# JiQi-da/Mixed-Graph-ADMM

Hardware: AMD Instinct MI355X
Metric: ADMM iters/sec x batch (sample-iterations/s) (higher is better)
Workload: dtype f32; 1 GPU; cfg2: PEMS04-shaped synthetic graph N=307 (path+chords, 340 edges), kNN k=4, T=24, t_in=12; batch_per_gpu=4096, global_batch=4096, ablation=None, graph=kNN-directed, max_cg_iter=100, parallelism=batch-sharded x1, no collective on the convergence path, final RCCL gather, all_finite=True

## Files before the change

include/mgadmm.h:

```cpp
#ifndef MGADMM_H
#define MGADMM_H

#include <stdint.h>

#ifdef __cplusplus
extern "C" {
#endif

typedef enum {
    MGADMM_OK = 0,
    MGADMM_ERR_INVALID = -1,
    MGADMM_ERR_HIP = -2,
    MGADMM_ERR_NONFINITE = -3,
    MGADMM_ERR_UNSUPPORTED = -4,
    MGADMM_ERR_NOMEM = -5
} mgadmm_status;

typedef enum { MGADMM_F32 = 0, MGADMM_F64 = 1 } mgadmm_dtype_t;

typedef enum {
    MGADMM_TEMPORAL_SPATIAL = 0,
    MGADMM_TEMPORAL_BAND = 1
} mgadmm_temporal_mode_t;

// ... 28 lines not shown
    const float* u_val;
    const int32_t* d_rowptr;
    const int32_t* d_col;
    const float* d_val;
    int32_t transpose_by_gather;
    int32_t q1_identity_t0;
    int32_t skip;
    const float* band_w;
    int32_t reorder;
    int32_t device;
} mgadmm_graph_desc;

typedef struct {
    double rho, rho_u, rho_d, mu_u, mu_d1, mu_d2;
    int32_t t_in;
    int32_t ablation;
    double cg_tol;
    int32_t max_cg_iter;
    double admm_tol;
    int32_t max_admm_iter;
    int32_t dtype;
    int32_t check_stop;
    int32_t path;
    int32_t record_cg_coeffs;
    int32_t cg_convergence;
    int32_t max_inner_iter;
    int32_t admm_convergence;
} mgadmm_params;

typedef struct {
    int32_t n_iters;
    double* metrics;
    double* delta_x_per_step;
    int32_t* cg_iters;
    double* metrics_per_sample;
    double* cg_alpha;
    double* cg_beta;
    int32_t* n_iters_per_sample;
} mgadmm_history;

typedef struct {
    void* zu; void* zd; void* phi; void* gamma; void* gamma_u; void* gamma_d;
} mgadmm_state;

typedef struct mgadmm_graph mgadmm_graph;
typedef struct mgadmm_solver mgadmm_solver;

const char* mgadmm_version(void);
const char* mgadmm_last_error(void);

int mgadmm_graph_create(const mgadmm_graph_desc* desc, mgadmm_graph** out);
int mgadmm_graph_destroy(mgadmm_graph* g);
int mgadmm_graph_transpose_nnz(const mgadmm_graph* g, int32_t* nnz);
int mgadmm_graph_get_transpose(const mgadmm_graph* g, int32_t* rowptr, int32_t* col, float* val);
int mgadmm_graph_get_perm(const mgadmm_graph* g, int32_t* perm);

int mgadmm_solver_create(mgadmm_graph* g, const mgadmm_params* p, int32_t max_batch, mgadmm_solver** out);
int mgadmm_solver_destroy(mgadmm_solver* s);
int mgadmm_solver_set_params(mgadmm_solver* s, const mgadmm_params* p);
typedef struct {
    const double *rho, *rho_u, *rho_d, *mu_u, *mu_d1, *mu_d2;
} mgadmm_sample_params;
int mgadmm_solver_set_sample_params(mgadmm_solver* s, const mgadmm_sample_params* sp, int32_t B);
int64_t mgadmm_solver_workspace_bytes(const mgadmm_solver* s);
int mgadmm_solver_path(const mgadmm_solver* s, int32_t B);

typedef enum {
    MGADMM_Q_LDS_OK = 0,
    MGADMM_Q_LDS_TPG = 1,
    MGADMM_Q_LDS_THREADS = 2,
    MGADMM_Q_LDS_BYTES = 3,
    MGADMM_Q_LDS_ROW_STRIDE = 4,
    MGADMM_Q_NNZ_U = 5,
    MGADMM_Q_NNZ_D = 6,
    MGADMM_Q_NNZ_DT = 7,
    MGADMM_Q_TILE_ROWS = 8,
    MGADMM_Q_LDS_UNIFORM = 9,
    MGADMM_Q_LDS_TAIL_PAIRS = 10,
    MGADMM_Q_LDS_LEAD = 11,
    MGADMM_Q_LDS_SLOTS = 12,
    MGADMM_Q_LDS_CHUNK = 13,
    MGADMM_Q_LDS_ROWS = 14,
    MGADMM_Q_CLDR_SLOTS = 15,
    MGADMM_Q_LDS_INSTANCE = 16
} mgadmm_query_t;
int mgadmm_solver_query(const mgadmm_solver* s, int32_t what, int64_t* out);

int mgadmm_apply(mgadmm_solver* s, int32_t op, const void* x, void* y, int32_t B, void* stream);
int mgadmm_lhs(mgadmm_solver* s, int32_t which, const void* x, const void* mask, void* y, int32_t B, void* stream);
int mgadmm_phi_direct(mgadmm_solver* s, const void* x, const void* gamma, void* phi, int32_t B, void* stream);
int mgadmm_initial_guess(mgadmm_solver* s, const void* y, void* x, int32_t B, void* stream);
int mgadmm_initial_interpolation(mgadmm_solver* s, const void* y, const void* mask, int32_t mask_is_f32,
                                 void* x, int32_t B, void* stream);
int mgadmm_cg(mgadmm_solver* s, int32_t which, const void* rhs, const void* x0, const void* mask, void* x,
              int32_t* iters, double* alpha, double* beta, int32_t B, void* stream);
int mgadmm_solve(mgadmm_solver* s, const void* y, const void* mask, int32_t mask_is_f32, int32_t B, void* x_out,
                 const mgadmm_state* state_out, mgadmm_history* hist, void* stream);

int mgadmm_solve_from(mgadmm_solver* s, const void* y, const void* mask, int32_t mask_is_f32, int32_t B, const void* x0,
                      const mgadmm_state* state_in, void* x_out, const mgadmm_state* state_out, mgadmm_history* hist,
                      void* stream);
int mgadmm_two_loops(mgadmm_solver* s, const void* y, const void* mask, int32_t mask_is_f32, int32_t B, void* x_out,
                     const mgadmm_state* state_out, mgadmm_history* hist, void* stream);

int mgadmm_knn_graph(int32_t n_nodes, int64_t n_edges, const int64_t* edges, const double* dists, int32_t k,
                     int32_t* nn_out, float* nd_out, int32_t device);
int mgadmm_weight_tables(int32_t n_nodes, int32_t k1, const int64_t* connect_list, const float* dist_list,
                         double u_sigma, double d_sigma, int32_t regularized, float* u_ew, float* d_ew,
                         double* sigmas_out, int32_t device);

int mgadmm_series_stats(const void* series, int64_t n_steps, int32_t n_cols, int32_t dtype, void* o_min, void* o_max,
                        void* o_mean, void* o_std, void* stream);
int mgadmm_series_affine(void* series, int64_t n_steps, int32_t n_cols, int32_t dtype, const void* shift, const void* scale,
                         const void* scale_lo, int32_t inverse, void* stream);
int mgadmm_gather_windows(const void* series, int64_t n_steps, int32_t n_cols, int32_t dtype, const int64_t* starts, int32_t B,
                          int32_t win, const float* mask, void* out, void* stream);

#define MGADMM_NPROF 4
int mgadmm_prof_begin(mgadmm_solver* s);
int mgadmm_prof_end(mgadmm_solver* s, int64_t* counts , double* total_ms ,
                    double* bytes );

#ifdef __cplusplus
}
#endif
#endif
```

mixed-graph-admm_amd/csrc/engine.h:

```cpp
#pragma once
#include <math.h>
#include <cmath>
#include <stdlib.h>
#include <string.h>

#include <algorithm>
#include <type_traits>

#include "common.h"
#include "cldr_tiles.h"
#include "stream_kernels.h"
#include "lds_args.h"
#include "lds_banks.h"
#include "lds_rows.h"

namespace {

struct LhsDef {
    int kind;
    int hth;
    double c1, c2;
};

enum VecId {
// ... 480 lines not shown
    }

    int set_sample_params(const mgadmm_sample_params* sp, int B) override {
        if (sp == nullptr || B == 0) {
            sp_B = 0;
            for (auto& v : sp_val) v.clear();
            return MGADMM_OK;
        }
        MG_REQUIRE(B >= 1 && B <= Bmax, "set_sample_params: batch %d outside [1, max_batch=%d]", B, Bmax);
        static const char* const names[6] = {"rho", "rho_u", "rho_d", "mu_u", "mu_d1", "mu_d2"};
        const double* const src[6] = {sp->rho, sp->rho_u, sp->rho_d, sp->mu_u, sp->mu_d1, sp->mu_d2};
        for (int f = 0; f < 6; ++f) {
            if (!src[f]) continue;
            for (int b = 0; b < B; ++b) {
                const double v = src[f][b];
                MG_REQUIRE(std::isfinite(v), "set_sample_params: %s[%d] is not finite", names[f], b);
                if (f < 3) MG_REQUIRE(v > 0.0, "set_sample_params: %s[%d] = %g, should be > 0", names[f], b, v);
                else MG_REQUIRE(v >= 0.0, "set_sample_params: %s[%d] = %g, should be >= 0", names[f], b, v);
            }
        }
        for (int f = 0; f < 6; ++f) {
            if (src[f]) sp_val[f].assign(src[f], src[f] + B);
            else sp_val[f].clear();
        }
        sp_B = B;
        MG_HIP(hipSetDevice(g->device));
        return upload_sample_params();
    }

    int upload_sample_params() {
        std::vector<LdsSampleParams> rec((size_t)sp_B);
        const double scalar[6] = {p.rho, p.rho_u, p.rho_d, p.mu_u, p.mu_d1, p.mu_d2};
        for (int b = 0; b < sp_B; ++b) {
            double w[6];
            for (int f = 0; f < 6; ++f) w[f] = sp_val[f].empty() ? scalar[f] : sp_val[f][(size_t)b];
            const LhsDef dx = lhs_def_of(MGADMM_LHS_X, p.ablation, w[0], w[1], w[2], w[3], w[5]);
            LdsSampleParams& r = rec[(size_t)b];
            r.cx1 = (float)dx.c1; r.cx2 = (float)dx.c2;
            r.rho = (float)w[0]; r.rho_u = (float)w[1]; r.rho_d = (float)w[2];
            r.mu_u = (float)w[3]; r.mu_d1 = (float)w[4]; r.mu_d2 = (float)w[5];
        }
        if (!d_sp) MG_HIP(hipMalloc(&d_sp, sizeof(LdsSampleParams) * (size_t)Bmax));
        MG_HIP(hipMemcpy(d_sp, rec.data(), sizeof(LdsSampleParams) * rec.size(), hipMemcpyHostToDevice));
        return MGADMM_OK;
    }

    int check_sample_params(int B) const {
        MG_REQUIRE(B == sp_B, "solve: the sample_params table holds %d samples, the solve has B = %d", sp_B, B);
        const char* why = nullptr;
        if (!std::is_same<S, float>::value) why = "float64 arithmetic runs on the streaming path";
        else if (p.path == MGADMM_PATH_STREAM) why = "path is MGADMM_PATH_STREAM";
        else if (p.cg_convergence == MGADMM_CG_BATCH_MAX) why = "cg_convergence batch_max runs on the streaming path";
        else if (!lds.ok) why = "the LDS-resident path cannot hold this graph (it needs T*N*8 B + tables <= 160 KiB and N*G <= 1024)";
        if (why) {
            mg_set_error("solve: sample_params (per-sample ADMM weights) are implemented by the LDS-resident float32 path only: %s", why);
            return MGADMM_ERR_UNSUPPORTED;
        }
        if (p.check_stop && p.admm_convergence == MGADMM_ADMM_WHOLE_BATCH) {
            mg_set_error("solve: sample_params with check_stop need admm_convergence per_sample (the whole_batch stop test would sum "
                         "the residuals of different problems); or run a fixed count with check_stop = 0");
            return MGADMM_ERR_UNSUPPORTED;
        }
        return MGADMM_OK;
    }

    int64_t workspace_bytes() const override { return ws_bytes; }
    int path_for(int) const override { return use_lds() ? MGADMM_PATH_LDS : MGADMM_PATH_STREAM; }
    bool use_lds() const { return lds.ok && p.path != MGADMM_PATH_STREAM && p.cg_convergence == MGADMM_CG_PER_SAMPLE; }
    int query(int what, int64_t* out) const override {
        switch (what) {
            case MGADMM_Q_LDS_OK: *out = lds.ok ? 1 : 0; break;
            case MGADMM_Q_LDS_TPG: *out = lds.TPG; break;
            case MGADMM_Q_LDS_THREADS: *out = lds.nthreads; break;
            case MGADMM_Q_LDS_BYTES: *out = (int64_t)lds.lds_bytes; break;
            case MGADMM_Q_LDS_ROW_STRIDE: *out = lds.TS; break;
            case MGADMM_Q_LDS_UNIFORM: *out = lds.uniform45; break;
            case MGADMM_Q_LDS_TAIL_PAIRS: *out = lds.tail_pairs; break;
            case MGADMM_Q_LDS_LEAD: *out = LDS_NLEAD; break;
            case MGADMM_Q_LDS_SLOTS: *out = lds.slots; break;
            case MGADMM_Q_LDS_CHUNK: *out = std::max(1, std::min(lds_chunk, LDS_MAXJ_POOL)); break;
            case MGADMM_Q_LDS_ROWS: *out = lds.NR; break;
            case MGADMM_Q_CLDR_SLOTS: *out = cldr_dev.state == 1 ? cl_gt : 0; break;
            case MGADMM_Q_LDS_INSTANCE: *out = lds_instance; break;
            case MGADMM_Q_NNZ_U: *out = g->hWu.nnz(); break;
            case MGADMM_Q_NNZ_D: *out = g->hWd.nnz(); break;
            case MGADMM_Q_NNZ_DT: *out = g->hWdT.nnz(); break;
            case MGADMM_Q_TILE_ROWS: {
                TileGeom tg;
                *out = make_tile_geom(make_geom(Bmax), tg) ? tg.R : 0;
                break;
            }
            default: mg_set_error("solver_query: unknown item %d", what); return MGADMM_ERR_INVALID;
        }
        return MGADMM_OK;
    }

    int prof_begin() override {
        MG_HIP(hipSetDevice(g->device));
        if (prof_ev.empty()) {
            prof_ev.resize(2 * PROF_POOL);
            for (auto& e : prof_ev) MG_HIP(hipEventCreateWithFlags(&e, hipEventDisableSystemFence));
            prof_tag.resize(PROF_POOL);
            prof_lb.resize(PROF_POOL);
            prof_ref.resize(PROF_POOL);
        }
        prof_used = 0;
        nact_cur = 0;
        nact_locked = false;
        for (int i = 0; i < MGADMM_NPROF; ++i) { prof_count[i] = 0; prof_bytes[i] = 0; }
        prof_on = true;
        return MGADMM_OK;
    }
    int prof_end(int64_t* counts, double* total_ms, double* bytes) override {
        prof_on = false;
        MG_HIP(hipDeviceSynchronize());
        double ms[MGADMM_NPROF] = {0}, by[MGADMM_NPROF] = {0};
        int64_t timed[MGADMM_NPROF] = {0};
        prof_noop = 0;
        for (size_t i = 0; i < prof_used; ++i) {
            float f = 0;
            MG_HIP(hipEventElapsedTime(&f, prof_ev[2 * i], prof_ev[2 * i + 1]));
            if (prof_ref[i] >= 0 && h_nact[prof_ref[i]] == 0) {
                prof_noop++;
                continue;
            }
            ms[prof_tag[i]] += f;
            by[prof_tag[i]] += prof_lb[i];
            timed[prof_tag[i]]++;
        }
        for (int i = 0; i < MGADMM_NPROF; ++i) {
            counts[i] = timed[i];
            total_ms[i] = ms[i];
            bytes[i] = by[i];
        }
        return MGADMM_OK;
    }
    inline bool prof_open(int tag, double bytes) {
        if (!prof_on) return false;
        prof_count[tag]++;
        prof_bytes[tag] += bytes;
        if (tag == 3 || prof_used >= (size_t)PROF_POOL) return false;
        prof_tag[prof_used] = tag;
        prof_lb[prof_used] = bytes;
        prof_ref[prof_used] = prof_cur_ref;
        (void)hipEventRecord(prof_ev[2 * prof_used], st);
        return true;
    }
    inline void prof_close() {
        (void)hipEventRecord(prof_ev[2 * prof_used + 1], st);
        prof_used++;
    }

    double pass_bytes(const Geom& q, int passes) const { return (double)passes * q.B * (double)T * N * sizeof(S); }
    double csr_bytes(const OpDesc& op) const {
        if (op.kind != OPK_SPATIAL) return 0.0;
        int nnz = 0;
        if (op.rowptr == g->Wu.rowptr) nnz = g->Wu.nnz;
        else if (op.rowptr == g->Wd.rowptr) nnz = g->Wd.nnz;
        else nnz = g->WdT.nnz;
        return (double)nnz * 8 + (double)(N + 1) * 4;
    }

    std::vector<const void*> lds_attr_done;
    int allow_dynamic_lds(const void* fn, int bytes) {
        for (const void* f : lds_attr_done)
            if (f == fn) return MGADMM_OK;
// ... 632 lines not shown
        } else {
            MG_TRY(pack(q, y, p.t_in, vec[V_Y]));
            MG_TRY(guess_internal(q, vec[V_Y], vec[xc]));
        }
        if (has_phi) {
            MG_TRY(fill(vec[V_GAM], ne, (S)0.1));
            MG_TRY(op_store(q, g->op_ldr(), vec[xc], vec[phc]));
        }
        const S rho = (S)p.rho, rho_u = (S)p.rho_u, rho_d = (S)p.rho_d;
        int n_done = 0;
        for (int o = 0; o < n_outer; ++o) {
            MG_TRY(fill(vec[V_GU], ne, (S)0.1));
            MG_TRY(fill(vec[V_GD], ne, (S)0.1));
            MG_HIP(hipMemcpyAsync(vec[zuc], vec[xc], ne * sizeof(S), hipMemcpyDeviceToDevice, st));
            MG_HIP(hipMemcpyAsync(vec[zdc], vec[xc], ne * sizeof(S), hipMemcpyDeviceToDevice, st));
            for (int in = 0; in < n_inner; ++in) {
                if (has_phi) {
                    MG_TRY(rows<EpiLin2>(q, op_none(), vec[V_GAM], nullptr, 3, 3, (const S*)vec[phc], vec[V_TMP], (S)1, rho));
                    MG_TRY(rows<EpiRhsX>(q, g->op_ldrt(), vec[V_TMP], nullptr, 2, has_zd ? 7 : 5, (const S*)vec[zuc],
                                         (const S*)vec[zdc], (const S*)vec[V_GU], (const S*)vec[V_GD], (const S*)vec[V_Y],
                                         vec[V_RHS], rho_u, rho_d, 1, has_zd ? 1 : 0));
                } else {
                    MG_TRY(rows<EpiRhsX>(q, op_none(), vec[zuc], nullptr, 3, 6, (const S*)vec[zuc], (const S*)vec[zdc],
                                         (const S*)vec[V_GU], (const S*)vec[V_GD], (const S*)vec[V_Y], vec[V_RHS], rho_u,
                                         rho_d, 0, 1));
                }
                int* it_base = d_cg_iters + ((size_t)o * n_inner + in) * 3 * q.Bp;
                MG_TRY(cg_internal(q, lhs_def(MGADMM_LHS_X), vec[V_RHS], vec[xc], m, vec[xn], it_base, false));
                MG_TRY(rows<EpiLin2>(q, op_none(), vec[V_GU], nullptr, 3, 3, (const S*)vec[xn], vec[V_RHS], (S)0.5, (S)(p.rho_u / 2)));
                MG_TRY(cg_internal(q, lhs_def(MGADMM_LHS_ZU), vec[V_RHS], vec[zuc], nullptr, vec[zun], it_base + q.Bp, false));
                if (has_zd) {
                    MG_TRY(rows<EpiLin2>(q, op_none(), vec[V_GD], nullptr, 3, 3, (const S*)vec[xn], vec[V_RHS], (S)0.5, (S)(p.rho_d / 2)));
                    MG_TRY(cg_internal(q, lhs_def(MGADMM_LHS_ZD), vec[V_RHS], vec[zdc], nullptr, vec[zdn], it_base + 2 * q.Bp, false));
                }
                const S* zd_now = has_zd ? vec[zdn] : vec[zdc];
                MG_TRY(rows<EpiDual>(q, op_none(), vec[xn], nullptr, 3, has_zd ? 11 : 6, (const S*)vec[xc], (const S*)vec[zun],
                                     (const S*)vec[zuc], zd_now, (const S*)vec[zdc], (const S*)vec[V_Y], m, vec[V_GU],
                                     vec[V_GD], rho_u, rho_d, has_zd ? 1 : 0, p.t_in));
                std::swap(xc, xn);
                std::swap(zuc, zun);
                if (has_zd) std::swap(zdc, zdn);
            }
            if (has_phi) {
                MG_TRY(rows<EpiPhi>(q, g->op_ldr(), vec[xc], nullptr, 2, 5, (const S*)vec[phc], vec[phn], vec[V_GAM], rho,
                                    (S)(p.mu_d1 / p.rho), 1));
                std::swap(phc, phn);
            }
            n_done = o + 1;
        }
        MG_TRY(unpack(q, vec[xc], x_out));
        if (state_out) {
            if (state_out->zu) MG_TRY(unpack(q, vec[zuc], state_out->zu));
            if (state_out->zd) MG_TRY(unpack(q, vec[zdc], state_out->zd));
            if (state_out->phi && has_phi) MG_TRY(unpack(q, vec[phc], state_out->phi));
            if (state_out->gamma && has_phi) MG_TRY(unpack(q, vec[V_GAM], state_out->gamma));
            if (state_out->gamma_u) MG_TRY(unpack(q, vec[V_GU], state_out->gamma_u));
            if (state_out->gamma_d) MG_TRY(unpack(q, vec[V_GD], state_out->gamma_d));
        }
        if (hist) {
            hist->n_iters = n_done;
            if (hist->cg_iters) {
                std::vector<int> tmp(rows_needed * 3 * q.Bp);
                MG_HIP(hipMemcpyAsync(tmp.data(), d_cg_iters, sizeof(int) * tmp.size(), hipMemcpyDeviceToHost, st));
                MG_HIP(hipStreamSynchronize(st));
                for (size_t r = 0; r < rows_needed * 3; ++r) memcpy(hist->cg_iters + r * B, tmp.data() + r * q.Bp, sizeof(int) * B);
            }
        }
        MG_HIP(hipMemcpyAsync(h_flag, d_nonfinite, sizeof(int), hipMemcpyDeviceToHost, st));
        MG_HIP(hipStreamSynchronize(st));
        if (h_flag[0]) {
            mg_set_error("two_loops: NaN/Inf met in the iterates (cf. the asserts of ADMM.py:432-504)");
            return MGADMM_ERR_NONFINITE;
        }
        return MGADMM_OK;
    }

    int plan_lds() {
        lds = LdsPlan();
        if (hipDeviceGetAttribute(&dev_cus, hipDeviceAttributeMultiprocessorCount, g->device) != hipSuccess) { (void)hipGetLastError(); dev_cus = 0; }
        if (!std::is_same<S, float>::value) return MGADMM_OK;
        const int tpgs[] = {1, 2, 3, 4, 6, 8, 12};
        int best = 0;
        const char* force = getenv("MGADMM_LDS_TPG");
        bool uni_graph = g->mode != MGADMM_TEMPORAL_BAND && !getenv("MGADMM_LDS_SB") && !getenv("MGADMM_LDS_RAGGED");
        for (int i = 0; i < N && uni_graph; ++i) {
            int ndiag = 0;
            for (int e = g->hWd.rowptr[i]; e < g->hWd.rowptr[i + 1]; ++e) ndiag += g->hWd.col[e] == i;
            uni_graph = g->hWu.rowptr[i + 1] - g->hWu.rowptr[i] == 4 && g->hWd.rowptr[i + 1] - g->hWd.rowptr[i] == 5 && ndiag == 1;
        }
        for (int tpg : tpgs) {
            if (T % tpg) continue;
            const int G = T / tpg;
            if ((long)N * G > 1024) continue;
            if (force && atoi(force) != tpg) continue;
            if (!best) best = tpg;
            if (uni_graph && !force && tpg == 8) best = 8;
        }
        if (!best) return MGADMM_OK;
        const bool band = g->mode == MGADMM_TEMPORAL_BAND;
        const int sb_env = getenv("MGADMM_LDS_SB") ? atoi(getenv("MGADMM_LDS_SB")) : 0;
        lds.TPG = best;
        lds.G = T / best;
        lds.nthreads = N * lds.G;
        lds.block = (lds.nthreads + 63) / 64 * 64;
        lds.maxt = (best == 12 && lds.block <= 640) ? 640 : 1024;
        lds.sb = (sb_env && ((best == 12 && lds.maxt == 640) || best == 8)) ? 1 : 0;
        const int NR = N + (lds.block - lds.nthreads);
        lds.NR = NR;
        lds.uniform45 = (!band && (best == 8 || best == 12) && !lds.sb && !getenv("MGADMM_LDS_RAGGED")) ? 1 : 0;
        for (int i = 0; i < N && lds.uniform45; ++i) {
            int ndiag = 0;
            for (int e = g->hWd.rowptr[i]; e < g->hWd.rowptr[i + 1]; ++e) ndiag += g->hWd.col[e] == i;
            if (g->hWu.rowptr[i + 1] - g->hWu.rowptr[i] != 4 || g->hWd.rowptr[i + 1] - g->hWd.rowptr[i] != 5 || ndiag != 1) lds.uniform45 = 0;
        }
        std::vector<float> diag_d(NR, 0.f), diag_t(NR, 0.f);
        auto strip_diag = [&](const HostCsr& h, std::vector<float>& dg) {
            HostCsr o;
            o.rowptr.push_back(0);
            for (int i = 0; i < N; ++i) {
                for (int e = h.rowptr[i]; e < h.rowptr[i + 1]; ++e) {
                    if (h.col[e] == i) dg[i] += h.val[e];
                    else { o.col.push_back(h.col[e]); o.val.push_back(h.val[e]); }
                }
                o.rowptr.push_back((int)o.col.size());
            }
            return o;
        };
        std::vector<int> deg_t(N, 0);
        if (!band)
            for (int i = 0; i < N; ++i)
                for (int e = g->hWdT.rowptr[i]; e < g->hWdT.rowptr[i + 1]; ++e) deg_t[i] += g->hWdT.col[e] != i;
        const int maxlen_t = N > 0 ? *std::max_element(deg_t.begin(), deg_t.end()) : 0;
        const int tp = band ? 0 : (std::max(0, maxlen_t - LDS_NLEAD) + 1) / 2;
        const int WT = LDS_NLEAD + 2 * tp;
        lds.tail_pairs = tp;
        const char* ro_env = getenv("MGADMM_LDS_ROW_ORDER");
        lds.row_order = (lds.uniform45 && tp <= 3) ? (ro_env ? std::max(0, std::min(atoi(ro_env), 2)) : (int)ldsrows::TAIL_CLASS) : 0;
        const ldsrows::Plan rows = ldsrows::make_plan(deg_t, lds.G, WT, lds.row_order, LDS_NLEAD);
        lds.npos_word = 0;
        if (lds.uniform45 && tp <= 3 && !ldsrows::pack_npos(rows, &lds.npos_word)) {
            mg_set_error("lds: row plan does not fit its launch word (%d waves)", (int)rows.npos.size());
            return MGADMM_ERR_INVALID;
        }
        const HostCsr Wu = lds.row_order ? ldsrows::relabel(g->hWu, rows) : g->hWu;
        const HostCsr Wd = lds.row_order ? ldsrows::relabel(g->hWd, rows) : g->hWd;
        const HostCsr WdT = lds.row_order ? ldsrows::relabel(g->hWdT, rows) : g->hWdT;
        const HostCsr hWdT_off = band ? HostCsr() : strip_diag(WdT, diag_t);
        const HostCsr hWd_tab = band ? HostCsr() : (lds.uniform45 ? strip_diag(Wd, diag_d) : Wd);
        auto with_ghosts = [&](const HostCsr& h, int fixed_len) {
            HostCsr o;
            o.rowptr.assign(h.rowptr.begin(), h.rowptr.begin() + N + 1);
            o.col = h.col; o.val = h.val;
            for (int r = N; r < NR; ++r) {
                for (int e = 0; e < fixed_len; ++e) { o.col.push_back(r); o.val.push_back(0.f); }
                o.rowptr.push_back((int)o.col.size());
            }
            return o;
        };
        const HostCsr hu = with_ghosts(Wu, lds.uniform45 ? 4 : 0);
        const HostCsr hd = band ? HostCsr() : with_ghosts(hWd_tab, lds.uniform45 ? 4 : 0);
        const int nu = hu.nnz(), nd = band ? 0 : hd.nnz();
        auto al4 = [](int v) { return (v + 3) & ~3; };
        int off = 0;
        lds.off_rp_u = off; off += NR + 1;
        lds.off_rp_d = off; off += NR + 1;
        off = al4(off);
        lds.off_en_u = off; off += 2 * nu;
        lds.off_en_d = off; off += 2 * nd;
        lds.off_lead_t = off; off += 2 * NR * LDS_NLEAD;
        off = al4(off);
        lds.off_tail_t = off; off += 2 * NR * 2 * tp + 4;
        const int tail_ints = off - lds.off_tail_t;
        lds.off_diag = off; off += 2 * NR;
        off += 8;
        lds.off_node = off; off += NR;
        lds.off_rown = off; off += N;
        lds.csr_ints = off;
        lds.lds_img0 = lds.uniform45 ? lds.off_tail_t : 0;
        lds.lds_img_ints = lds.uniform45 ? tail_ints : lds.off_diag;
        int ts = (T + 3) / 4 * 4;
        if (((ts / 4) & 1) == 0) ts += 4;
        auto bytes_for = [&](int stride, int slots) {
            const size_t LN = (size_t)NR * stride;
            return sizeof(float) * ((lds.sb ? 1 : 2) * LN + ((4 - (LN & 3)) & 3) + 32 + 16 * 12 + (size_t)slots * 2 * lds.block * best)
                   + sizeof(int) * (size_t)lds.lds_img_ints;
        };
        if (bytes_for(ts, 0) > 160 * 1024) ts = T;
        lds.TS = ts;
        if (bytes_for(ts, 0) > 160 * 1024) { lds = LdsPlan(); return MGADMM_OK; }
        lds.slots = (lds.uniform45 && !getenv("MGADMM_LDS_NOSLOTS") && bytes_for(ts, 1) <= 160 * 1024) ? 1 : 0;
        lds.lds_bytes = bytes_for(ts, lds.slots);
        std::vector<int> img(off, 0);
// ... 383 lines not shown
```

mixed-graph-admm_amd/csrc/lds_kernels.h:

```cpp
#pragma once
#include "common.h"
#include "lds_args.h"



template <int CTRL, int ROW_MASK>
__device__ __forceinline__ float dpp_step(float v) {
    const int moved = __builtin_amdgcn_update_dpp(0, __float_as_int(v), CTRL, ROW_MASK, 0xf, false);
    return v + __int_as_float(moved);
}
__device__ __forceinline__ float wave_sum(float v) {
    v = dpp_step<0x111, 0xf>(v);
    v = dpp_step<0x112, 0xf>(v);
    v = dpp_step<0x114, 0xf>(v);
    v = dpp_step<0x118, 0xf>(v);
    asm("s_nop 1\n\tv_add_f32_dpp %0, %0, %0 row_bcast:15 row_mask:0xa bank_mask:0xf\n\t"
        "s_nop 1\n\tv_add_f32_dpp %0, %0, %0 row_bcast:31 row_mask:0xc bank_mask:0xf\n\ts_nop 1" : "+v"(v));
    return __int_as_float(__builtin_amdgcn_readlane(__float_as_int(v), 63));
}

struct BlockRed {
    float* red;
    int par;
    int lane, wave, nwaves;
    __device__ __forceinline__ double sum(float v) {
        v = wave_sum(v);
        float* buf = red + par * 16;
        if (lane == 0) buf[wave] = v;
        __syncthreads();
        const float4 a = reinterpret_cast<const float4*>(buf)[0], b = reinterpret_cast<const float4*>(buf)[1],
                     c = reinterpret_cast<const float4*>(buf)[2], d = reinterpret_cast<const float4*>(buf)[3];
        const float sx = (a.x + b.x) + (c.x + d.x), sy = (a.y + b.y) + (c.y + d.y);
        const float sz = (a.z + b.z) + (c.z + d.z), sw = (a.w + b.w) + (c.w + d.w);
        const double s = (double)((sx + sy) + (sz + sw));
        par ^= 1;
        return s;
    }
    __device__ __forceinline__ float sumf(float v) {
        v = wave_sum(v);
        float* buf = red + par * 16;
        if (lane == 0) buf[wave] = v;
        __syncthreads();
        float t = buf[lane & 15];
        t = dpp_step<0x111, 0xf>(t);
        t = dpp_step<0x112, 0xf>(t);
        t = dpp_step<0x114, 0xf>(t);
        t = dpp_step<0x118, 0xf>(t);
        par ^= 1;
        return __int_as_float(__builtin_amdgcn_readlane(__float_as_int(t), 15));
    }
};

typedef float lds_f4 __attribute__((ext_vector_type(4)));
template <int TPG>
__device__ __forceinline__ void lds_load(const float* p, float (&v)[TPG]) {
    if constexpr (TPG % 4 == 0) {
#pragma unroll
        for (int j = 0; j < TPG / 4; ++j) {
            const lds_f4 q = static_cast<const lds_f4*>(__builtin_assume_aligned(p, 16))[j];
            v[4 * j] = q.x; v[4 * j + 1] = q.y; v[4 * j + 2] = q.z; v[4 * j + 3] = q.w;
        }
    } else if constexpr (TPG % 2 == 0) {
#pragma unroll
        for (int j = 0; j < TPG / 2; ++j) {
            const float2 q = reinterpret_cast<const float2*>(p)[j];
            v[2 * j] = q.x; v[2 * j + 1] = q.y;
        }
    } else {
#pragma unroll
        for (int j = 0; j < TPG; ++j) v[j] = p[j];
    }
}
template <int TPG>
__device__ __forceinline__ void lds_store(float* p, const float (&v)[TPG]) {
    if constexpr (TPG % 4 == 0) {
#pragma unroll
        for (int j = 0; j < TPG / 4; ++j) {
            lds_f4 q;
            q.x = v[4 * j]; q.y = v[4 * j + 1]; q.z = v[4 * j + 2]; q.w = v[4 * j + 3];
            static_cast<lds_f4*>(__builtin_assume_aligned(p, 16))[j] = q;
        }
    } else if constexpr (TPG % 2 == 0) {
#pragma unroll
        for (int j = 0; j < TPG / 2; ++j) reinterpret_cast<float2*>(p)[j] = make_float2(v[2 * j], v[2 * j + 1]);
    } else {
#pragma unroll
        for (int j = 0; j < TPG; ++j) p[j] = v[j];
    }
}

__device__ __forceinline__ float ldg(const float* base, unsigned boff) {
    const __attribute__((address_space(1))) char* g = (const __attribute__((address_space(1))) char*)base;
    return *reinterpret_cast<const __attribute__((address_space(1))) float*>(g + boff);
}
__device__ __forceinline__ void stg(float* base, unsigned boff, float v) {
    __attribute__((address_space(1))) char* g = (__attribute__((address_space(1))) char*)base;
    *reinterpret_cast<__attribute__((address_space(1))) float*>(g + boff) = v;
}
#define MG_REQ_FENCE() asm volatile("" ::: "memory")
#define MG_PIN_S(x) asm volatile("" : "+s"(x))
#define MG_PIN_V(x) asm volatile("" : "+v"(x))

typedef int lds_i4 __attribute__((ext_vector_type(4)));
template <typename P>
__device__ __forceinline__ P* scalar_ptr(P* p) {
    const unsigned long long u = (unsigned long long)p;
    const unsigned lo = __builtin_amdgcn_readfirstlane((unsigned)u), hi = __builtin_amdgcn_readfirstlane((unsigned)(u >> 32));
    return (P*)(((unsigned long long)hi << 32) | lo);
}
typedef float f2 __attribute__((ext_vector_type(2)));
__device__ __forceinline__ f2 mk2(float a, float b) { f2 r; r.x = a; r.y = b; return r; }
template <int TPG>
__device__ __forceinline__ void axpy(float a, const float (&x)[TPG], float (&y)[TPG]) {
    if constexpr (TPG % 2 == 0) {
#pragma unroll
        for (int j = 0; j < TPG / 2; ++j) {
            const f2 r = __builtin_elementwise_fma(mk2(a, a), mk2(x[2 * j], x[2 * j + 1]), mk2(y[2 * j], y[2 * j + 1]));
            y[2 * j] = r.x; y[2 * j + 1] = r.y;
        }
// ... 298 lines not shown
#pragma unroll
        for (int k = 0; k < TPG; ++k) l[k] = ((k > 0 || t0 > 0 || q1) ? self[k] : 0.f) - acc[k];
    }
    template <int SH>
    __device__ __forceinline__ void put(float* DST, const float (&v)[TPG]) const {
        if constexpr (SH == 0 || BAND) {
            lds_store<TPG>(DST + own(), v);
        } else {
            float* row = DST + i * TS + t0 - SH;
            constexpr int K0 = SH < 0 ? 3 : 1;
            constexpr int NG = TPG % 4 == 0 ? (TPG - K0) / 4 : 0;
#pragma unroll
            for (int j = 0; j < NG; ++j) {
                lds_f4 q;
                q.x = v[K0 + 4 * j]; q.y = v[K0 + 4 * j + 1]; q.z = v[K0 + 4 * j + 2]; q.w = v[K0 + 4 * j + 3];
                *static_cast<lds_f4*>(__builtin_assume_aligned(row + K0 + 4 * j, 16)) = q;
            }
#pragma unroll
            for (int k = 0; k < TPG; ++k) {
                if (k >= K0 && k < K0 + 4 * NG) continue;
                const bool ok = SH < 0 ? (k < TPG - 1 || t0 + TPG < T) : (k > 0 || t0 > 0);
                if (ok) row[k] = v[k];
            }
            if (SH < 0 && t0 == 0) DST[i * TS] = 0.f;
            if (SH > 0 && t0 + TPG == T) DST[i * TS + T - 1] = 0.f;
        }
    }
    __device__ __forceinline__ void puts(float* DST, const float (&v)[TPG]) const {
        if (active) {
            unsigned o = so0;
            MG_PIN_V(o);
            __attribute__((address_space(1))) char* g = (__attribute__((address_space(1))) char*)DST;
            if constexpr (TPG % 4 == 0) {
#pragma unroll
                for (int j = 0; j < TPG / 4; ++j) {
                    lds_f4 q;
                    q.x = v[4 * j]; q.y = v[4 * j + 1]; q.z = v[4 * j + 2]; q.w = v[4 * j + 3];
                    *reinterpret_cast<__attribute__((address_space(1))) lds_f4*>(g + o + 16 * j) = q;
                }
            } else {
#pragma unroll
                for (int k = 0; k < TPG; ++k) *reinterpret_cast<__attribute__((address_space(1))) float*>(g + o + 4 * k) = v[k];
            }
        }
    }
    __device__ __forceinline__ void putg(float* DST, const float (&v)[TPG]) const {
        if (active) {
            unsigned o0 = glb0();
            MG_PIN_V(o0);
#pragma unroll
            for (int k = 0; k < TPG; ++k) stg(DST, o0 + kN4[k], v[k]);
        }
    }
};

template <int TPG>
__device__ __forceinline__ void slot_put(float* S, int tid, int nthr, const float (&v)[TPG]) {
    if constexpr (TPG % 4 == 0) {
#pragma unroll
        for (int j = 0; j < TPG / 4; ++j) {
            lds_f4 q;
            q.x = v[4 * j]; q.y = v[4 * j + 1]; q.z = v[4 * j + 2]; q.w = v[4 * j + 3];
            static_cast<lds_f4*>(__builtin_assume_aligned(S, 16))[j * nthr + tid] = q;
        }
    } else {
#pragma unroll
        for (int k = 0; k < TPG; ++k) S[k * nthr + tid] = v[k];
    }
}
template <int TPG>
__device__ __forceinline__ void slot_get(const float* S, int tid, int nthr, float (&v)[TPG]) {
    if constexpr (TPG % 4 == 0) {
#pragma unroll
        for (int j = 0; j < TPG / 4; ++j) {
            const lds_f4 q = static_cast<const lds_f4*>(__builtin_assume_aligned(S, 16))[j * nthr + tid];
            v[4 * j] = q.x; v[4 * j + 1] = q.y; v[4 * j + 2] = q.z; v[4 * j + 3] = q.w;
        }
    } else {
#pragma unroll
        for (int k = 0; k < TPG; ++k) v[k] = S[k * nthr + tid];
    }
}

template <int TPG, bool BAND, int KIND, bool SB, int NU, int ND, int TP>
__device__ __forceinline__ float lds_apply(LdsCtx<TPG, BAND, NU, ND, TP>& c, const float (&v)[TPG], float (&av)[TPG], const float (&dc)[TPG],
                                           float c2, typename LdsCtx<TPG, BAND, NU, ND, TP>::Rows& R) {
    typedef LdsCtx<TPG, BAND, NU, ND, TP> Ctx;
    if constexpr (Ctx::UNI) {
        if (KIND == 1) {
#pragma unroll
            for (int u = 0; u < Ctx::NDO; ++u) MG_PIN_V(R.d[u]);
#pragma unroll
            for (int u = 0; u < LDS_NLEAD; ++u) MG_PIN_V(R.t[u]);
        } else if (KIND == 2) {
#pragma unroll
            for (int u = 0; u < NU; ++u) MG_PIN_V(R.u[u]);
        }
    }
    if (KIND == 1 && !BAND) MG_PIN_V(c.wdiag);
    float l[TPG];
#pragma unroll
    for (int k = 0; k < TPG; ++k) l[k] = 0.f;
    if (KIND == 1) {
        if constexpr (BAND) {
            float q[TPG];
            c.op_ldr(c.P, v, q, R);
            if (SB) __syncthreads();
            c.template put<+1>(c.Q, q);
            __syncthreads();
            c.op_ldrt(c.Q, q, l, R);
        } else {
            float q[TPG];
            {
                float acc[TPG];
                c.mul_wd(c.P, acc, R, v);
                const bool has_next = c.t0 + TPG < c.T;
                float vnext;
                if constexpr (TPG % 4 == 0) vnext = static_cast<const lds_f4*>(__builtin_assume_aligned(c.P + c.own() + (has_next ? TPG : 0), 16))[0].x;
                else vnext = c.P[c.own() + (has_next ? TPG : 0)];
#pragma unroll
                for (int k = 0; k + 1 < TPG; ++k) q[k] = v[k + 1] - acc[k];
                q[TPG - 1] = (has_next ? vnext : acc[TPG - 1]) - acc[TPG - 1];
            }
            if (SB) __syncthreads();
            lds_store<TPG>(c.Q + c.own(), q);
            __syncthreads();
            {
                float acc[TPG];
                c.mul_wdt(c.Q, acc, R, q);
                const bool has_prev = c.t0 > 0;
                float qprev;
                if constexpr (TPG % 4 == 0) qprev = static_cast<const lds_f4*>(__builtin_assume_aligned(c.Q + c.own() - (has_prev ? 4 : 0), 16))[0].w;
                else qprev = c.Q[c.own() - (has_prev ? 1 : 0)];
                l[0] = (has_prev ? qprev : 0.f) - acc[0];
#pragma unroll
                for (int k = 1; k < TPG; ++k) l[k] = q[k - 1] - acc[k];
            }
        }
    } else if (KIND == 2) {
        c.op_lu(c.P, v, l, R);
    }
    if constexpr (TPG % 2 == 0) {
#pragma unroll
        for (int j = 0; j < TPG / 2; ++j) {
            f2 r = mk2(dc[2 * j], dc[2 * j + 1]) * mk2(v[2 * j], v[2 * j + 1]);
            if (KIND != 0) r = __builtin_elementwise_fma(mk2(c2, c2), mk2(l[2 * j], l[2 * j + 1]), r);
            av[2 * j] = r.x; av[2 * j + 1] = r.y;
        }
    } else {
#pragma unroll
        for (int k = 0; k < TPG; ++k) av[k] = (KIND == 0) ? dc[k] * v[k] : __builtin_fmaf(c2, l[k], dc[k] * v[k]);
    }
    return dot<TPG>(v, av);
}
template <int TPG, bool BAND, int NU, int ND, int TP>
__device__ __forceinline__ void lds_diag(const LdsCtx<TPG, BAND, NU, ND, TP>& c, const float* dg, int hth, int t_in, float c1, float (&dc)[TPG]) {
    if (dg) {
        unsigned o = c.glb0();
        MG_PIN_V(o);
        float mv[TPG];
#pragma unroll
        for (int k = 0; k < TPG; ++k) mv[k] = ldg(dg, o + c.kN4[k]);
        MG_REQ_FENCE();
#pragma unroll
        for (int k = 0; k < TPG; ++k) dc[k] = (c.active ? mv[k] : 0.f) + c1;
    } else {
        const int lim = hth ? t_in - c.t0 : 0;
#pragma unroll
        for (int k = 0; k < TPG; ++k) dc[k] = (k < lim ? 1.f : 0.f) + c1;
    }
}

template <int TPG, bool BAND, int KIND, bool SB, int NU, int ND, int TP>
__device__ __forceinline__ int lds_cg(LdsCtx<TPG, BAND, NU, ND, TP>& c, BlockRed& br, float (&x)[TPG], const float (&rhs)[TPG], const float* dmask,
                      int hth, int t_in, float c1, float c2, int max_cg, double tol2, float* ah, float* bh, int Bp,
                      int* nonfinite, typename LdsCtx<TPG, BAND, NU, ND, TP>::Rows& R) {
    float r[TPG], pv[TPG], av[TPG], dc[TPG];
#pragma unroll
    for (int k = 0; k < TPG; ++k) { pv[k] = x[k]; r[k] = 0.f; }
    c.template put<0>(c.P, pv);
    lds_diag<TPG, BAND, NU, ND, TP>(c, dmask, hth, t_in, c1, dc);
    float rr = 0.f;
    int iters = -1;
    bool done = false, init = true;
    for (int it = -1; it < max_cg && !done; ++it) {
        __syncthreads();
        const float part = lds_apply<TPG, BAND, KIND, SB, NU, ND, TP>(c, pv, av, dc, c2, R);
        if (init) {
            init = false;
            if (dmask != nullptr) lds_diag<TPG, BAND, NU, ND, TP>(c, nullptr, hth, t_in, c1, dc);
#pragma unroll
            for (int k = 0; k < TPG; ++k) {
                r[k] = rhs[k] - av[k];
                pv[k] = r[k];
            }
            rr = br.sumf(dot<TPG>(r, r));
            c.template put<0>(c.P, pv);
            continue;
        }
        const float pAp = br.sumf(part);
        const float alpha = rr * __builtin_amdgcn_rcpf(pAp);
        axpy<TPG>(alpha, pv, x);
        axpy<TPG>(-alpha, av, r);
        const float rrn = br.sumf(dot<TPG>(r, r));
        const float beta = rrn * __builtin_amdgcn_rcpf(rr);
        rr = rrn;
        if (ah != nullptr && threadIdx.x == 0) {
            ah[(size_t)it * Bp] = alpha;
            bh[(size_t)it * Bp] = beta;
        }
        const bool bad = !(fabsf(rrn) <= 3.0e38f);
        const bool conv = (double)rrn < tol2;
        if (bad && threadIdx.x == 0) *nonfinite = 1;
        if (conv && !bad) iters = it + 1;
        done = bad || conv;
        xpby<TPG>(r, beta, pv);
        c.template put<0>(c.P, pv);
    }
    return iters;
}

#ifdef MGADMM_LDS_PER_SAMPLE_PARAMS
#define MG_LDS_KERNEL k_admm_lds_pp
#define MG_LDS_PS true
#define MG_LDS_PSTOP_ON(args) ((args).pstop != nullptr)
#if defined(__HIP_DEVICE_COMPILE__)
#define MG_LDS_W(field) (((const LdsSampleParams __attribute__((address_space(4)))*)a.sp)[b].field)
#else
#define MG_LDS_W(field) (a.sp[b].field)
#endif
#else
#ifdef MGADMM_LDS_PER_SAMPLE_STOP
#define MG_LDS_KERNEL k_admm_lds_ps
#define MG_LDS_PS true
#else
#define MG_LDS_KERNEL k_admm_lds
#define MG_LDS_PS false
#endif
#define MG_LDS_PSTOP_ON(args) true
#define MG_LDS_W(field) (a.field)
#endif
template <int TPG, bool BAND, int MAXT, bool SB, int NU = 0, int ND = 0, bool SLOTS = false, int TP = -1>
__global__ __launch_bounds__(MAXT, (SB && MAXT == 640) ? 5 : 1) void MG_LDS_KERNEL(LdsArgs a_in) {
    constexpr bool PS = MG_LDS_PS;
    constexpr bool ENTG = NU > 0 && ND > 0;
    constexpr int NMRED = 12;
    extern __shared__ __align__(16) unsigned char lds_raw[];
    float* P = reinterpret_cast<float*>(lds_raw);
    const int LN = a_in.NR * a_in.TS;
    float* Q = SB ? P : P + LN;
    float* red = Q + LN + ((4 - (LN & 3)) & 3);
    float* mred = red + 32;
    float* slot0 = mred + 16 * NMRED;
    const int nthr = (int)blockDim.x;
    float* slot1 = slot0 + (SLOTS ? nthr * TPG : 0);
    int* img = reinterpret_cast<int*>(slot1 + (SLOTS ? nthr * TPG : 0));
    int tid = threadIdx.x;
    int b = blockIdx.x;
    if (a_in.stop != nullptr && *a_in.stop != 0) return;
    if constexpr (PS) {
        if (MG_LDS_PSTOP_ON(a_in) && a_in.pstop[b] != 0) return;
    }
    if (a_in.stagger_ticks > 0 && b < a_in.stagger_wgs) {
        const unsigned long long wait = (unsigned long long)a_in.stagger_ticks * (unsigned)b / (unsigned)a_in.stagger_wgs;
        const unsigned long long t_in0 = wall_clock64();
        while (wall_clock64() - t_in0 < wait) __builtin_amdgcn_s_sleep(16);
    }
    {
        const int* src = a_in.csr + a_in.lds_img0;
        const int nimg = a_in.lds_img_ints;
        for (int k0 = tid; k0 < nimg; k0 += 8 * nthr) {
            int wv[8];
#pragma unroll
            for (int u = 0; u < 8; ++u) {
                const int k = k0 + u * nthr;
                wv[u] = src[k < nimg ? k : nimg - 1];
            }
#pragma unroll
            for (int u = 0; u < 8; ++u) {
                const int k = k0 + u * nthr;
                if (k < nimg) img[k] = wv[u];
            }
        }
// ... 720 lines not shown
```

mixed-graph-admm_amd/mgadmm/_lib.py:

```python
import ctypes as C
import os

import torch

_HERE = os.path.dirname(os.path.abspath(__file__))
LIB_PATH = os.environ.get("MGADMM_LIB") or os.path.join(_HERE, "libmgadmm.so")

OK, ERR_INVALID, ERR_HIP, ERR_NONFINITE, ERR_UNSUPPORTED, ERR_NOMEM = 0, -1, -2, -3, -4, -5
F32, F64 = 0, 1
TEMPORAL_SPATIAL, TEMPORAL_BAND = 0, 1
OP_LU, OP_LDR, OP_LDRT, OP_CLDR, OP_LN = 0, 1, 2, 3, 4
CG_PER_SAMPLE, CG_BATCH_MAX = 0, 1
ADMM_WHOLE_BATCH, ADMM_PER_SAMPLE = 0, 1
LHS_X, LHS_ZU, LHS_ZD = 0, 1, 2
ABLATIONS = {"None": 0, "DGTV": 1, "DGLR": 2, "UT": 3}
PATH_AUTO, PATH_STREAM, PATH_LDS = 0, 1, 2
NMETRIC = 11
(M_XSHIFT, M_PRI_ZU, M_DUAL_ZU, M_PRI_PHI, M_DUAL_PHI, M_PRI_ZD, M_DUAL_ZD, M_GLR, M_DGTV, M_DGLR,
 M_RECOVER) = range(11)
NPROF = 4
(Q_LDS_OK, Q_LDS_TPG, Q_LDS_THREADS, Q_LDS_BYTES, Q_LDS_ROW_STRIDE, Q_NNZ_U, Q_NNZ_D, Q_NNZ_DT, Q_TILE_ROWS, Q_LDS_UNIFORM,
 Q_LDS_TAIL_PAIRS, Q_LDS_LEAD, Q_LDS_SLOTS, Q_LDS_CHUNK, Q_LDS_ROWS, Q_CLDR_SLOTS, Q_LDS_INSTANCE) = range(17)

_i32p = C.POINTER(C.c_int32)
_f32p = C.POINTER(C.c_float)
_f64p = C.POINTER(C.c_double)


class GraphDesc(C.Structure):
    _fields_ = [
        ("n_nodes", C.c_int32), ("T", C.c_int32), ("temporal_mode", C.c_int32),
        ("u_rowptr", _i32p), ("u_col", _i32p), ("u_val", _f32p),
        ("d_rowptr", _i32p), ("d_col", _i32p), ("d_val", _f32p),
        ("transpose_by_gather", C.c_int32), ("q1_identity_t0", C.c_int32),
        ("skip", C.c_int32), ("band_w", _f32p),
        ("reorder", C.c_int32), ("device", C.c_int32),
    ]


class Params(C.Structure):
    _fields_ = [
        ("rho", C.c_double), ("rho_u", C.c_double), ("rho_d", C.c_double),
        ("mu_u", C.c_double), ("mu_d1", C.c_double), ("mu_d2", C.c_double),
        ("t_in", C.c_int32), ("ablation", C.c_int32),
        ("cg_tol", C.c_double), ("max_cg_iter", C.c_int32),
        ("admm_tol", C.c_double), ("max_admm_iter", C.c_int32),
        ("dtype", C.c_int32), ("check_stop", C.c_int32), ("path", C.c_int32),
        ("record_cg_coeffs", C.c_int32), ("cg_convergence", C.c_int32), ("max_inner_iter", C.c_int32),
        ("admm_convergence", C.c_int32),
    ]


class History(C.Structure):
    _fields_ = [
        ("n_iters", C.c_int32),
        ("metrics", _f64p), ("delta_x_per_step", _f64p), ("cg_iters", _i32p),
        ("metrics_per_sample", _f64p), ("cg_alpha", _f64p), ("cg_beta", _f64p),
        ("n_iters_per_sample", _i32p),
    ]


class State(C.Structure):
    _fields_ = [("zu", C.c_void_p), ("zd", C.c_void_p), ("phi", C.c_void_p), ("gamma", C.c_void_p),
                ("gamma_u", C.c_void_p), ("gamma_d", C.c_void_p)]


class SampleParams(C.Structure):
    _fields_ = [("rho", _f64p), ("rho_u", _f64p), ("rho_d", _f64p), ("mu_u", _f64p), ("mu_d1", _f64p), ("mu_d2", _f64p)]


_vp = C.c_void_p
SYMBOLS = {
    "mgadmm_version": (C.c_char_p, []),
    "mgadmm_last_error": (C.c_char_p, []),
    "mgadmm_graph_create": (C.c_int, [C.POINTER(GraphDesc), C.POINTER(_vp)]),
    "mgadmm_graph_destroy": (C.c_int, [_vp]),
    "mgadmm_graph_transpose_nnz": (C.c_int, [_vp, _i32p]),
    "mgadmm_graph_get_transpose": (C.c_int, [_vp, _i32p, _i32p, _f32p]),
    "mgadmm_graph_get_perm": (C.c_int, [_vp, _i32p]),
    "mgadmm_solver_create": (C.c_int, [_vp, C.POINTER(Params), C.c_int32, C.POINTER(_vp)]),
    "mgadmm_solver_destroy": (C.c_int, [_vp]),
    "mgadmm_solver_set_params": (C.c_int, [_vp, C.POINTER(Params)]),
    "mgadmm_solver_set_sample_params": (C.c_int, [_vp, C.POINTER(SampleParams), C.c_int32]),
    "mgadmm_solver_workspace_bytes": (C.c_int64, [_vp]),
    "mgadmm_solver_path": (C.c_int, [_vp, C.c_int32]),
    "mgadmm_solver_query": (C.c_int, [_vp, C.c_int32, C.POINTER(C.c_int64)]),
    "mgadmm_apply": (C.c_int, [_vp, C.c_int32, _vp, _vp, C.c_int32, _vp]),
    "mgadmm_lhs": (C.c_int, [_vp, C.c_int32, _vp, _vp, _vp, C.c_int32, _vp]),
    "mgadmm_phi_direct": (C.c_int, [_vp, _vp, _vp, _vp, C.c_int32, _vp]),
    "mgadmm_initial_guess": (C.c_int, [_vp, _vp, _vp, C.c_int32, _vp]),
    "mgadmm_initial_interpolation": (C.c_int, [_vp, _vp, _vp, C.c_int32, _vp, C.c_int32, _vp]),
    "mgadmm_cg": (C.c_int, [_vp, C.c_int32, _vp, _vp, _vp, _vp, _i32p, _f64p, _f64p, C.c_int32, _vp]),
    "mgadmm_solve": (C.c_int, [_vp, _vp, _vp, C.c_int32, C.c_int32, _vp, C.POINTER(State), C.POINTER(History), _vp]),
    "mgadmm_solve_from": (C.c_int, [_vp, _vp, _vp, C.c_int32, C.c_int32, _vp, C.POINTER(State), _vp, C.POINTER(State), C.POINTER(History), _vp]),
    "mgadmm_two_loops": (C.c_int, [_vp, _vp, _vp, C.c_int32, C.c_int32, _vp, C.POINTER(State), C.POINTER(History), _vp]),
    "mgadmm_knn_graph": (C.c_int, [C.c_int32, C.c_int64, C.POINTER(C.c_int64), _f64p, C.c_int32, _i32p, _f32p, C.c_int32]),
    "mgadmm_weight_tables": (C.c_int, [C.c_int32, C.c_int32, C.POINTER(C.c_int64), _f32p, C.c_double, C.c_double, C.c_int32,
                                       _f32p, _f32p, _f64p, C.c_int32]),
    "mgadmm_series_stats": (C.c_int, [_vp, C.c_int64, C.c_int32, C.c_int32, _vp, _vp, _vp, _vp, _vp]),
    "mgadmm_series_affine": (C.c_int, [_vp, C.c_int64, C.c_int32, C.c_int32, _vp, _vp, _vp, C.c_int32, _vp]),
    "mgadmm_gather_windows": (C.c_int, [_vp, C.c_int64, C.c_int32, C.c_int32, _vp, C.c_int32, C.c_int32, _vp, _vp, _vp]),
    "mgadmm_prof_begin": (C.c_int, [_vp]),
    "mgadmm_prof_end": (C.c_int, [_vp, C.POINTER(C.c_int64), _f64p, _f64p]),
}

# ... 50 lines not shown
```

Before: 3.001 million ADMM sample-iterations/s.

## Fold CG pAp reduction into the existing LDS barrier of the uniform apply

In the uniform LDS CG path for the X system, each wave now publishes its partial of p^T A p before the barrier that already exists inside the operator apply. The partial is computed algebraically as c2·q·q + dc·v². The block total is then read after that barrier, which removes the separate block-reduction barrier per CG iteration. It also disables the uniform path when the graph uses transpose-by-gather and adds a query that reports the barrier count. The rewritten quadratic form changes floating-point rounding relative to the direct dot(v, Av).

Result: faster. 3.080 million ADMM sample-iterations/s (median of 6 runs) (+2.7%).

```diff
diff --git a/include/mgadmm.h b/include/mgadmm.h
--- a/include/mgadmm.h
+++ b/include/mgadmm.h
@@ -134,6 +134,7 @@
     MGADMM_Q_LDS_CHUNK = 13,
     MGADMM_Q_LDS_ROWS = 14,
     MGADMM_Q_CLDR_SLOTS = 15,
+    MGADMM_Q_LDS_CG_BARRIERS = 17,
     MGADMM_Q_LDS_INSTANCE = 16
 } mgadmm_query_t;
 int mgadmm_solver_query(const mgadmm_solver* s, int32_t what, int64_t* out);
diff --git a/mixed-graph-admm_amd/csrc/engine.h b/mixed-graph-admm_amd/csrc/engine.h
--- a/mixed-graph-admm_amd/csrc/engine.h
+++ b/mixed-graph-admm_amd/csrc/engine.h
@@ -586,6 +586,7 @@
             case MGADMM_Q_LDS_ROWS: *out = lds.NR; break;
             case MGADMM_Q_CLDR_SLOTS: *out = cldr_dev.state == 1 ? cl_gt : 0; break;
             case MGADMM_Q_LDS_INSTANCE: *out = lds_instance; break;
+            case MGADMM_Q_LDS_CG_BARRIERS: *out = !lds.ok ? 0 : (lds.uniform45 ? 3 : 4 + lds.sb); break;
             case MGADMM_Q_NNZ_U: *out = g->hWu.nnz(); break;
             case MGADMM_Q_NNZ_D: *out = g->hWd.nnz(); break;
             case MGADMM_Q_NNZ_DT: *out = g->hWdT.nnz(); break;
@@ -1384,7 +1385,7 @@
         const int tpgs[] = {1, 2, 3, 4, 6, 8, 12};
         int best = 0;
         const char* force = getenv("MGADMM_LDS_TPG");
-        bool uni_graph = g->mode != MGADMM_TEMPORAL_BAND && !getenv("MGADMM_LDS_SB") && !getenv("MGADMM_LDS_RAGGED");
+        bool uni_graph = g->mode != MGADMM_TEMPORAL_BAND && !g->transpose_by_gather && !getenv("MGADMM_LDS_SB") && !getenv("MGADMM_LDS_RAGGED");
         for (int i = 0; i < N && uni_graph; ++i) {
             int ndiag = 0;
             for (int e = g->hWd.rowptr[i]; e < g->hWd.rowptr[i + 1]; ++e) ndiag += g->hWd.col[e] == i;
@@ -1409,7 +1410,7 @@
         lds.sb = (sb_env && ((best == 12 && lds.maxt == 640) || best == 8)) ? 1 : 0;
         const int NR = N + (lds.block - lds.nthreads);
         lds.NR = NR;
-        lds.uniform45 = (!band && (best == 8 || best == 12) && !lds.sb && !getenv("MGADMM_LDS_RAGGED")) ? 1 : 0;
+        lds.uniform45 = (!band && !g->transpose_by_gather && (best == 8 || best == 12) && !lds.sb && !getenv("MGADMM_LDS_RAGGED")) ? 1 : 0;
         for (int i = 0; i < N && lds.uniform45; ++i) {
             int ndiag = 0;
             for (int e = g->hWd.rowptr[i]; e < g->hWd.rowptr[i + 1]; ++e) ndiag += g->hWd.col[e] == i;
diff --git a/mixed-graph-admm_amd/csrc/lds_kernels.h b/mixed-graph-admm_amd/csrc/lds_kernels.h
--- a/mixed-graph-admm_amd/csrc/lds_kernels.h
+++ b/mixed-graph-admm_amd/csrc/lds_kernels.h
@@ -35,6 +35,21 @@
         const double s = (double)((sx + sy) + (sz + sw));
         par ^= 1;
         return s;
+    }
+    __device__ __forceinline__ void publish(float v) {
+        v = wave_sum(v);
+        float* buf = red + par * 16;
+        if (lane == 0) buf[wave] = v;
+    }
+    __device__ __forceinline__ float total() { return total_of(total_read()); }
+    __device__ __forceinline__ float total_read() const { return red[par * 16 + (lane & 15)]; }
+    __device__ __forceinline__ float total_of(float t) {
+        t = dpp_step<0x111, 0xf>(t);
+        t = dpp_step<0x112, 0xf>(t);
+        t = dpp_step<0x114, 0xf>(t);
+        t = dpp_step<0x118, 0xf>(t);
+        par ^= 1;
+        return __int_as_float(__builtin_amdgcn_readlane(__float_as_int(t), 15));
     }
     __device__ __forceinline__ float sumf(float v) {
         v = wave_sum(v);
@@ -499,10 +514,14 @@
     }
 }
 
+template <int KIND, bool BAND, bool SB, bool UNI>
+constexpr bool lds_fold_v = KIND == 1 && UNI && !BAND && !SB;
 template <int TPG, bool BAND, int KIND, bool SB, int NU, int ND, int TP>
-__device__ __forceinline__ float lds_apply(LdsCtx<TPG, BAND, NU, ND, TP>& c, const float (&v)[TPG], float (&av)[TPG], const float (&dc)[TPG],
-                                           float c2, typename LdsCtx<TPG, BAND, NU, ND, TP>::Rows& R) {
+__device__ __forceinline__ float lds_apply(LdsCtx<TPG, BAND, NU, ND, TP>& c, BlockRed& br, const float (&v)[TPG], float (&av)[TPG],
+                                           const float (&dc)[TPG], float c2, typename LdsCtx<TPG, BAND, NU, ND, TP>::Rows& R) {
     typedef LdsCtx<TPG, BAND, NU, ND, TP> Ctx;
+    constexpr bool FOLD = lds_fold_v<KIND, BAND, SB, Ctx::UNI>;
+    float vAv = 0.f;
     if constexpr (Ctx::UNI) {
         if (KIND == 1) {
 #pragma unroll
@@ -541,7 +560,18 @@
             }
             if (SB) __syncthreads();
             lds_store<TPG>(c.Q + c.own(), q);
+            if constexpr (FOLD) {
+                float vv[TPG];
+#pragma unroll
+                for (int j = 0; j < TPG / 2; ++j) {
+                    const f2 t = mk2(v[2 * j], v[2 * j + 1]) * mk2(v[2 * j], v[2 * j + 1]);
+                    vv[2 * j] = t.x; vv[2 * j + 1] = t.y;
+                }
+                br.publish(__builtin_fmaf(c2, dot<TPG>(q, q), dot<TPG>(dc, vv)));
+            }
             __syncthreads();
+            float slot = 0.f;
+            if constexpr (FOLD) slot = br.total_read();
             {
                 float acc[TPG];
                 c.mul_wdt(c.Q, acc, R, q);
@@ -553,6 +583,10 @@
 #pragma unroll
                 for (int k = 1; k < TPG; ++k) l[k] = q[k - 1] - acc[k];
             }
+            if constexpr (FOLD) {
+                MG_PIN_V(slot);
+                vAv = br.total_of(slot);
+            }
         }
     } else if (KIND == 2) {
         c.op_lu(c.P, v, l, R);
@@ -568,7 +602,8 @@
 #pragma unroll
         for (int k = 0; k < TPG; ++k) av[k] = (KIND == 0) ? dc[k] * v[k] : __builtin_fmaf(c2, l[k], dc[k] * v[k]);
     }
-    return dot<TPG>(v, av);
+    if constexpr (FOLD) return vAv;
+    else return dot<TPG>(v, av);
 }
 template <int TPG, bool BAND, int NU, int ND, int TP>
 __device__ __forceinline__ void lds_diag(const LdsCtx<TPG, BAND, NU, ND, TP>& c, const float* dg, int hth, int t_in, float c1, float (&dc)[TPG]) {
@@ -602,7 +637,7 @@
     bool done = false, init = true;
     for (int it = -1; it < max_cg && !done; ++it) {
         __syncthreads();
-        const float part = lds_apply<TPG, BAND, KIND, SB, NU, ND, TP>(c, pv, av, dc, c2, R);
+        const float part = lds_apply<TPG, BAND, KIND, SB, NU, ND, TP>(c, br, pv, av, dc, c2, R);
         if (init) {
             init = false;
             if (dmask != nullptr) lds_diag<TPG, BAND, NU, ND, TP>(c, nullptr, hth, t_in, c1, dc);
@@ -615,7 +650,9 @@
             c.template put<0>(c.P, pv);
             continue;
         }
-        const float pAp = br.sumf(part);
+        float pAp;
+        if constexpr (lds_fold_v<KIND, BAND, SB, LdsCtx<TPG, BAND, NU, ND, TP>::UNI>) pAp = part;
+        else pAp = br.sumf(part);
         const float alpha = rr * __builtin_amdgcn_rcpf(pAp);
         axpy<TPG>(alpha, pv, x);
         axpy<TPG>(-alpha, av, r);
diff --git a/mixed-graph-admm_amd/mgadmm/_lib.py b/mixed-graph-admm_amd/mgadmm/_lib.py
--- a/mixed-graph-admm_amd/mgadmm/_lib.py
+++ b/mixed-graph-admm_amd/mgadmm/_lib.py
@@ -20,7 +20,7 @@
  M_RECOVER) = range(11)
 NPROF = 4
 (Q_LDS_OK, Q_LDS_TPG, Q_LDS_THREADS, Q_LDS_BYTES, Q_LDS_ROW_STRIDE, Q_NNZ_U, Q_NNZ_D, Q_NNZ_DT, Q_TILE_ROWS, Q_LDS_UNIFORM,
- Q_LDS_TAIL_PAIRS, Q_LDS_LEAD, Q_LDS_SLOTS, Q_LDS_CHUNK, Q_LDS_ROWS, Q_CLDR_SLOTS, Q_LDS_INSTANCE) = range(17)
+ Q_LDS_TAIL_PAIRS, Q_LDS_LEAD, Q_LDS_SLOTS, Q_LDS_CHUNK, Q_LDS_ROWS, Q_CLDR_SLOTS, Q_LDS_INSTANCE, Q_LDS_CG_BARRIERS) = range(18)
 
 _i32p = C.POINTER(C.c_int32)
 _f32p = C.POINTER(C.c_float)
```
